# ssmit1986/BayesianInference

Measured on AMD Instinct MI355X. Metric: GP log-marg-lik evals/sec at N=32768, d=8; Cholesky TFLOP/s vs fp64 peak, higher is better.
Workload: dtype f64

## Files before the change

bayesianinference_amd/csrc/gp_trsv.h:

```cpp
#pragma once
#include "gp_kernels.h"

namespace gphip {

constexpr int TRSV_MAXR = 4;
constexpr int TRSV_CHAIN = 8;
constexpr int TRSV_SPIN_LIMIT = 1 << 24;
#ifndef TRSV_TILE_BACKOFF
#define TRSV_TILE_BACKOFF 6
#endif

template <typename T>
struct TrsvArgs {
    const T* A; int R128;
    const T* W;
    const T* P;
    const T* B;
    T* X;
    T* Xc;
    T* S;
    long ldx;
    int nt, nrhs, back;
    int dbg;
    unsigned int* ticket;
    long long* trace;
    int* abort_flag;
};

template <typename T> struct TrsvBits;
template <> struct TrsvBits<double> {
    typedef unsigned long long u;
    static __device__ __forceinline__ bool pending(double v) { return __double_as_longlong(v) == -1ll; }
};
template <> struct TrsvBits<float> {
    typedef unsigned int u;
    static __device__ __forceinline__ bool pending(float v) { return __float_as_int(v) == -1; }
};

template <typename T, int MODE, typename Src>
__device__ __forceinline__ void trsv_fetch(Src src, int nrhs, T* dst, int lane, int* abort_flag) {
    T va[2 * TRSV_MAXR];
    int spins = 0;
    auto give_up = [&]() -> bool {
        if ((++spins & 255) != 0) return false;
        if (__hip_atomic_load(abort_flag, __ATOMIC_RELAXED, __HIP_MEMORY_SCOPE_AGENT) != 0) return true;
        if (spins > TRSV_SPIN_LIMIT) { __hip_atomic_store(abort_flag, 1, __ATOMIC_RELAXED, __HIP_MEMORY_SCOPE_AGENT); return true; }
        return false;
    };
    auto load_set = [&](T (&v)[2 * TRSV_MAXR]) {
#pragma unroll
        for (int r = 0; r < TRSV_MAXR; ++r)
            if (r < nrhs) {
                const T* p = src(r);
                if (MODE == 0) {
                    v[2 * r] = p[lane];
                    v[2 * r + 1] = p[64 + lane];
                } else {
                    v[2 * r] = __hip_atomic_load(p + lane, __ATOMIC_RELAXED, __HIP_MEMORY_SCOPE_AGENT);
                    v[2 * r + 1] = __hip_atomic_load(p + 64 + lane, __ATOMIC_RELAXED, __HIP_MEMORY_SCOPE_AGENT);
                }
            }
    };
    auto complete = [&](const T (&v)[2 * TRSV_MAXR]) -> bool {
        bool bad = false;
#pragma unroll
        for (int r = 0; r < TRSV_MAXR; ++r)
            if (r < nrhs) bad = bad || TrsvBits<T>::pending(v[2 * r]) || TrsvBits<T>::pending(v[2 * r + 1]);
        return __all(!bad);
    };
    load_set(va);
    if (MODE != 0) {
        while (__builtin_expect(!complete(va), 0)) {
            if (MODE == 1) __builtin_amdgcn_s_sleep(TRSV_TILE_BACKOFF);
            load_set(va);
            if (give_up()) break;
        }
    }
#pragma unroll
    for (int r = 0; r < TRSV_MAXR; ++r)
        if (r < nrhs) {
            dst[r * TB + lane] = va[2 * r];
            dst[r * TB + 64 + lane] = va[2 * r + 1];
        }
}

template <typename T, bool BACK> struct TrsvBlk {
    static constexpr int NC = BACK ? 4 : 8, NR = BACK ? 8 : 4;
    T a[BACK ? 4 : 8][BACK ? 8 : 4];
};
template <typename T, bool BACK>
__device__ __forceinline__ void trsv_load_tile(TrsvBlk<T, BACK>& m, const T* __restrict__ tile, int lo, int ob) {
    constexpr int NC = TrsvBlk<T, BACK>::NC, NR = TrsvBlk<T, BACK>::NR;
    const int c0 = BACK ? 4 * ob : 8 * lo, r0 = BACK ? 8 * lo : 4 * ob;
#pragma unroll
    for (int cc = 0; cc < NC; ++cc) {
        const T* p = tile + (long)(c0 + cc) * TB + r0;
#pragma unroll
        for (int rr = 0; rr < NR; ++rr) m.a[cc][rr] = p[rr];
    }
}

template <typename T, bool BACK>
__device__ __forceinline__ void trsv_settle(TrsvBlk<T, BACK>& m) {
    asm volatile("s_waitcnt vmcnt(0)" ::: "memory");
#pragma unroll
    for (int cc = 0; cc < TrsvBlk<T, BACK>::NC; ++cc)
#pragma unroll
        for (int rr = 0; rr < TrsvBlk<T, BACK>::NR; ++rr) asm volatile("" : "+v"(m.a[cc][rr]));
}

template <int CTRL> __device__ __forceinline__ double trsv_dpp(double v) {
    const int lo = __builtin_amdgcn_update_dpp(0, __double2loint(v), CTRL, 0xF, 0xF, true);
    const int hi = __builtin_amdgcn_update_dpp(0, __double2hiint(v), CTRL, 0xF, 0xF, true);
    return __hiloint2double(hi, lo);
}
template <int CTRL> __device__ __forceinline__ float trsv_dpp(float v) {
    return __int_as_float(__builtin_amdgcn_update_dpp(0, __float_as_int(v), CTRL, 0xF, 0xF, true));
}
template <typename T> __device__ __forceinline__ T trsv_row16_sum(T v) {
    v += trsv_dpp<0xB1>(v);
    v += trsv_dpp<0x4E>(v);
    v += trsv_dpp<0x141>(v);
    v += trsv_dpp<0x140>(v);
    return v;
}

template <typename T, bool BACK>
__device__ __forceinline__ void trsv_matvec(const TrsvBlk<T, BACK>& m, const T* x, int lo, T (&y)[4]) {
    T xv[8];
#pragma unroll
    for (int k = 0; k < 8; ++k) xv[k] = x[lo * 8 + k];
    if constexpr (!BACK) {
#pragma unroll
        for (int rr = 0; rr < 4; ++rr) {
            T acc = (T)0;
#pragma unroll
            for (int cc = 0; cc < 8; ++cc) acc = __builtin_fma(m.a[cc][rr], xv[cc], acc);
            y[rr] = acc;
        }
    } else {
#pragma unroll
        for (int cc = 0; cc < 4; ++cc) {
            T acc = (T)0;
#pragma unroll
            for (int rr = 0; rr < 8; ++rr) acc = __builtin_fma(m.a[cc][rr], xv[rr], acc);
            y[cc] = acc;
        }
    }
#pragma unroll
    for (int k = 0; k < 4; ++k) y[k] = trsv_row16_sum(y[k]);
}

template <typename T, bool BACK> struct TrsvHalf {
    static constexpr int NC = BACK ? 2 : 8, NR = BACK ? 8 : 2;
    T a[BACK ? 2 : 8][BACK ? 8 : 2];
};
template <typename T, bool BACK>
__device__ __forceinline__ void trsv_load_half(TrsvHalf<T, BACK>& m, const T* __restrict__ tile, int lo, int ob, int hf) {
    constexpr int NC = TrsvHalf<T, BACK>::NC, NR = TrsvHalf<T, BACK>::NR;
    const int c0 = BACK ? 64 * hf + 2 * ob : 8 * lo, r0 = BACK ? 8 * lo : 64 * hf + 2 * ob;
#pragma unroll
    for (int cc = 0; cc < NC; ++cc) {
        const T* p = tile + (long)(c0 + cc) * TB + r0;
#pragma unroll
        for (int rr = 0; rr < NR; ++rr) m.a[cc][rr] = p[rr];
    }
}
template <typename T, bool BACK>
__device__ __forceinline__ void trsv_settle_half(TrsvHalf<T, BACK>& m) {
    asm volatile("s_waitcnt vmcnt(0)" ::: "memory");
#pragma unroll
    for (int cc = 0; cc < TrsvHalf<T, BACK>::NC; ++cc)
#pragma unroll
        for (int rr = 0; rr < TrsvHalf<T, BACK>::NR; ++rr) asm volatile("" : "+v"(m.a[cc][rr]));
}
template <typename T, bool BACK>
__device__ __forceinline__ void trsv_half_fma(const TrsvHalf<T, BACK>& m, const T* x, int lo, bool negate, T (&y)[2]) {
    T xv[8];
#pragma unroll
    for (int k = 0; k < 8; ++k) xv[k] = negate ? -x[lo * 8 + k] : x[lo * 8 + k];
    if constexpr (!BACK) {
#pragma unroll
        for (int cc = 0; cc < 8; ++cc)
#pragma unroll
            for (int rr = 0; rr < 2; ++rr) y[rr] = __builtin_fma(m.a[cc][rr], xv[cc], y[rr]);
    } else {
#pragma unroll
        for (int rr = 0; rr < 8; ++rr)
#pragma unroll
            for (int cc = 0; cc < 2; ++cc) y[cc] = __builtin_fma(m.a[cc][rr], xv[rr], y[cc]);
    }
}

template <typename T>
__global__ __launch_bounds__(256) void trsv_prep_kernel(const T* __restrict__ A, int R128, const T* __restrict__ W, T* __restrict__ P, int nt, int back) {
    __shared__ T As[16][TB + 4], Bs[16][TB + 4];
    const int b = blockIdx.x, gap = (int)blockIdx.y + 1, tid = threadIdx.x, tx = tid & 15, ty = tid >> 4;
    if (back ? b > nt - 1 - gap : b < gap) return;
    P += (long)blockIdx.y * nt * TS;
    const T* Lt = A + tile_index(back ? b + gap : b, back ? b : b - gap, R128) * TS;
    const T* Wb = W + (long)b * TS;
    const T* Am = back ? Lt : Wb;
    const T* Bm = back ? Wb : Lt;
    T c[8][8];
#pragma unroll
    for (int i = 0; i < 8; ++i)
#pragma unroll
        for (int j = 0; j < 8; ++j) c[i][j] = (T)0;
    for (int k0 = 0; k0 < TB; k0 += 16) {
        for (int idx = tid; idx < 16 * TB; idx += 256) {
            const int kk = idx >> 7, r = idx & 127;
            As[kk][r] = Am[(long)(k0 + kk) * TB + r];
        }
        for (int idx = tid; idx < 16 * TB; idx += 256) {
            const int cc = idx >> 4, kk = idx & 15;
            Bs[kk][cc] = Bm[(long)cc * TB + k0 + kk];
        }
        __syncthreads();
#pragma unroll 4
        for (int kk = 0; kk < 16; ++kk) {
            T av[8], bv[8];
#pragma unroll
            for (int i = 0; i < 8; ++i) { av[i] = As[kk][8 * ty + i]; bv[i] = Bs[kk][8 * tx + i]; }
#pragma unroll
            for (int i = 0; i < 8; ++i)
#pragma unroll
                for (int j = 0; j < 8; ++j) c[i][j] = __builtin_fma(av[i], bv[j], c[i][j]);
        }
        __syncthreads();
    }
    T* Pb = P + (long)b * TS;
#pragma unroll
    for (int j = 0; j < 8; ++j)
#pragma unroll
        for (int i = 0; i < 8; ++i) Pb[(long)(8 * tx + j) * TB + 8 * ty + i] = c[i][j];
}

constexpr int TRSV_THREADS = 512;

template <typename T, bool BACK>
__global__ __launch_bounds__(TRSV_THREADS, 1) void trsv_dataflow_kernel(TrsvArgs<T> g) {
    constexpr int NC = TrsvBlk<T, BACK>::NC, NR = TrsvBlk<T, BACK>::NR;
    extern __shared__ double trsv_lds_raw[];
    __shared__ unsigned int s_q;
    T* xs = reinterpret_cast<T*>(trsv_lds_raw);
    T* ss = xs + TRSV_MAXR * TB;
    const int tid = threadIdx.x, lane = tid & 63, wave = tid >> 6;
    const int lo = tid & 15, ob = tid >> 4;
    const int nt = g.nt, nrhs = g.nrhs;
    auto blk = [&](int K) { return BACK ? nt - 1 - K : K; };
    const T* Xpoll = (g.dbg & 64) ? g.Xc : g.X;
    auto sslot = [&](int I, int K) { return g.S + ((long)I * (I - 1) / 2 + K) * nrhs * TB; };
    auto ltile = [&](int I, int K) {
        const int bi = blk(I), bk = blk(K);
        return g.A + tile_index(bi > bk ? bi : bk, bi > bk ? bk : bi, g.R128) * TS;
    };

    if ((int)blockIdx.x < 2 * TRSV_CHAIN) {
        TrsvHalf<T, BACK> w, p1, p2;
        const int hf = (int)blockIdx.x & 1;
        T* xs2 = ss + TRSV_MAXR * TB;
        for (int K = (int)blockIdx.x >> 1; K < nt; K += TRSV_CHAIN) {
            const int b = blk(K);
            long long* tr = (g.trace && hf == 0) ? g.trace + (long)K * 8 : nullptr;
            long long st[8];
            auto stamp = [&](int k) { if (tr) st[k] = wall_clock64(); };
            stamp(0);
            if (tr) st[6] = clock64();
            trsv_load_half<T, BACK>(w, g.W + (long)b * TS, lo, ob, hf);
            if (K > 0) trsv_load_half<T, BACK>(p1, g.P + (long)b * TS, lo, ob, hf);
            if (K > 1) trsv_load_half<T, BACK>(p2, g.P + ((long)nt + b) * TS, lo, ob, hf);
            trsv_settle_half(w);
            trsv_settle_half(p1);
            trsv_settle_half(p2);
            if (wave == 1) {
                if (K >= 3 && !(g.dbg & 1)) trsv_fetch<T, 2>([&](int r) { return sslot(K, K - 3) + (long)r * TB; }, nrhs, ss, lane, g.abort_flag);
                else trsv_fetch<T, 0>([&](int r) { return g.B + (long)r * g.ldx + (long)b * TB; }, nrhs, ss, lane, g.abort_flag);
            }
            if (wave == 2 && K > 1)
                trsv_fetch<T, 1>([&](int r) { return g.X + (long)r * g.ldx + (long)blk(K - 2) * TB; }, nrhs, xs2, lane, g.abort_flag);
            __syncthreads();
            stamp(2);
            T y[TRSV_MAXR][2];
#pragma unroll
            for (int r = 0; r < TRSV_MAXR; ++r) {
                y[r][0] = y[r][1] = (T)0;
                if (r < nrhs) {
                    trsv_half_fma<T, BACK>(w, ss + r * TB, lo, false, y[r]);
                    if (K > 1) trsv_half_fma<T, BACK>(p2, xs2 + r * TB, lo, true, y[r]);
                }
            }
            stamp(3);
            if (wave == 0 && K > 0)
                trsv_fetch<T, 2>([&](int r) { return g.Xc + (long)r * g.ldx + (long)blk(K - 1) * TB; }, nrhs, xs, lane, g.abort_flag);
            stamp(1);
            __syncthreads();
            stamp(4);
#pragma unroll
            for (int r = 0; r < TRSV_MAXR; ++r)
                if (r < nrhs) {
                    if (K > 0) trsv_half_fma<T, BACK>(p1, xs + r * TB, lo, true, y[r]);
                    y[r][0] = trsv_row16_sum(y[r][0]);
                    y[r][1] = trsv_row16_sum(y[r][1]);
                    if (lo == 0) {
                        T* oc = g.Xc + (long)r * g.ldx + (long)b * TB + 64 * hf + 2 * ob;
                        T* ox = g.X + (long)r * g.ldx + (long)b * TB + 64 * hf + 2 * ob;
                        __hip_atomic_store(oc, y[r][0], __ATOMIC_RELAXED, __HIP_MEMORY_SCOPE_AGENT);
                        __hip_atomic_store(oc + 1, y[r][1], __ATOMIC_RELAXED, __HIP_MEMORY_SCOPE_AGENT);
                        __hip_atomic_store(ox, y[r][0], __ATOMIC_RELAXED, __HIP_MEMORY_SCOPE_AGENT);
                        __hip_atomic_store(ox + 1, y[r][1], __ATOMIC_RELAXED, __HIP_MEMORY_SCOPE_AGENT);
                    }
                }
            stamp(5);
            if (tr) {
                st[7] = clock64();
                if (tid == 0)
                    for (int k = 0; k < 8; ++k) tr[k] = st[k];
            }
            __syncthreads();
        }
        return;
    }

    auto tile_out = [&](const TrsvBlk<T, BACK>& cur, int I, int K) {
        T* out = sslot(I, K);
        for (int r = 0; r < nrhs; ++r) {
            T y[4];
            trsv_matvec<T, BACK>(cur, xs + r * TB, lo, y);
            if (lo == 0) {
#pragma unroll
                for (int k = 0; k < 4; ++k)
                    __hip_atomic_store(out + (long)r * TB + ob * 4 + k, ss[r * TB + ob * 4 + k] - y[k], __ATOMIC_RELAXED, __HIP_MEMORY_SCOPE_AGENT);
            }
        }
    };
    if ((int)blockIdx.x < 3 * TRSV_CHAIN) {
        TrsvBlk<T, BACK> cur;
        for (int K = (int)blockIdx.x - 2 * TRSV_CHAIN; K + 3 < nt; K += TRSV_CHAIN) {
            const int I = K + 3;
            trsv_load_tile<T, BACK>(cur, ltile(I, K), lo, ob);
            trsv_settle(cur);
            if (wave == 0) trsv_fetch<T, 1>([&](int r) { return g.X + (long)r * g.ldx + (long)blk(K) * TB; }, nrhs, xs, lane, g.abort_flag);
            if (wave == 1) {
                if (K > 0) trsv_fetch<T, 1>([&](int r) { return sslot(I, K - 1) + (long)r * TB; }, nrhs, ss, lane, g.abort_flag);
                else trsv_fetch<T, 0>([&](int r) { return g.B + (long)r * g.ldx + (long)blk(I) * TB; }, nrhs, ss, lane, g.abort_flag);
            }
            __syncthreads();
            tile_out(cur, I, K);
            __syncthreads();
        }
        return;
    }

    if (nt < 5) return;
    const long ntasks = (long)(nt - 4) * (nt - 3) / 2;
    auto take = [&]() -> long {
        __syncthreads();
        if (tid == 0) s_q = atomicAdd(g.ticket, 1u) + 1u;
        __syncthreads();
        return (long)s_q;
    };
    auto decode = [&](long q, int& I, int& K) {
        const double bq = (double)(2 * nt - 7);
        int k = (int)((bq - sqrt(bq * bq - 8.0 * (double)q)) * 0.5);
        if (k < 0) k = 0;
        if (k > nt - 5) k = nt - 5;
        while (k + 1 <= nt - 5 && (long)(k + 1) * (nt - 4) - (long)(k + 1) * k / 2 <= q) ++k;
        while (k > 0 && (long)k * (nt - 4) - (long)k * (k - 1) / 2 > q) --k;
        K = __builtin_amdgcn_readfirstlane(k);
        I = __builtin_amdgcn_readfirstlane(k + 4 + (int)(q - ((long)k * (nt - 4) - (long)k * (k - 1) / 2)));
    };
    TrsvBlk<T, BACK> ta, tb;
    long q = take();
    if (q >= ntasks) return;
    int I, K;
    decode(q, I, K);
    trsv_load_tile<T, BACK>(ta, ltile(I, K), lo, ob);
    auto process = [&](TrsvBlk<T, BACK>& cur, TrsvBlk<T, BACK>& nxt) -> bool {
        const long qn = take();
        int In = 0, Kn = 0;
        if (qn < ntasks) {
            decode(qn, In, Kn);
            trsv_load_tile<T, BACK>(nxt, ltile(In, Kn), lo, ob);
        }
        if (wave == 0) trsv_fetch<T, 1>([&](int r) { return Xpoll + (long)r * g.ldx + (long)blk(K) * TB; }, nrhs, xs, lane, g.abort_flag);
        if (wave == 1) {
            if (K > 0) trsv_fetch<T, 1>([&](int r) { return sslot(I, K - 1) + (long)r * TB; }, nrhs, ss, lane, g.abort_flag);
            else trsv_fetch<T, 0>([&](int r) { return g.B + (long)r * g.ldx + (long)blk(I) * TB; }, nrhs, ss, lane, g.abort_flag);
        }
        trsv_settle(cur);
        trsv_settle(nxt);
        __syncthreads();
        tile_out(cur, I, K);
        I = In; K = Kn;
        return qn < ntasks;
    };
    for (;;) {
        if (!process(ta, tb)) return;
        if (!process(tb, ta)) return;
    }
}

template <typename T>
__global__ void rows_to_vblock_kernel(const T* __restrict__ rows, int mc, long npad, T* __restrict__ V, long mpad) {
    const long j = (long)blockIdx.x * blockDim.x + threadIdx.x;
    if (j >= npad) return;
    for (long t = 0; t < mpad; ++t) V[j * mpad + t] = t < mc ? rows[t * npad + j] : (T)0;
}
template <typename T>
__global__ void vblock_to_rows_kernel(const T* __restrict__ V, long mpad, int mc, long npad, T* __restrict__ rows) {
    const long j = (long)blockIdx.x * blockDim.x + threadIdx.x;
    if (j >= npad) return;
    for (int t = 0; t < mc; ++t) rows[(long)t * npad + j] = V[j * mpad + t];
}

template <typename T>
__global__ __launch_bounds__(256) void w128_to_w64_kernel(const T* __restrict__ W128, T* __restrict__ W64, long slot_stride = 0) {
    const int j = blockIdx.x, b = j >> 1, q = j & 1;
    const T* src = W128 + (long)blockIdx.y * slot_stride + (long)b * TS + (long)(q * 64) * TB + q * 64;
    T* dst = W64 + (long)blockIdx.y * slot_stride + (long)j * 4096;
    for (int idx = threadIdx.x; idx < 4096; idx += 256) {
        const int c = idx >> 6, r = idx & 63;
        dst[idx] = src[(long)c * TB + r];
    }
}

constexpr size_t trsv_lds_bytes(size_t es) { return (size_t)(3 * TRSV_MAXR * TB) * es; }

}
```

bayesianinference_amd/csrc/gphip.hip:

```cpp
#include "gp_kernels.h"
#include "gp_trsv.h"
#include "rccl_dyn.h"
#include "rtc_dyn.h"

#include <hip/hip_ext.h>

#include <algorithm>
#include <chrono>
#include <cctype>
#include <cmath>
#include <cstdio>
#include <cstdlib>
#include <cstring>
#include <mutex>
#include <string>
#include <vector>

#include "../../include/gphip.h"

using namespace gphip;

namespace {

constexpr double LOG_TWO_PI = 1.8378770664093454835606594728112;
// ... 99 lines not shown
    Buf dA, dXs, dW;
    Buf dDinv;
    Buf dW64;
    unsigned long w64_gen = ~0ul;
    Buf dLT, dW64T;
    unsigned long lt_gen = ~0ul;
    Buf dInvEll, dSlotp, dPartial, dRes, dInfo;
    Buf hInvEll, hSlotp, hRes, hInfo;
    int panel = 4, profile = 0, swizzle = 1, max_slots = 256, lookahead = 1;
    int supertile = 2;
    int latency_gemm = 1;
    static constexpr int latency_tiles = 256;
    int latency_max_nt = 48;
    int dataflow = 1, dataflow_max_nt = 96;
    int dataflow_max_slots = -1;
    int dataflow_max_tasks = 34000;
    int dataflow_fine_nt = 96;
    int panel_left = -1;
    int fuse_option = 1;
    int grad_potri = 1;
    int grad_batch_slots = 0;
    int grad_batch_max_n = 7168;
    int grad_batch_last = 0, grad_batch_route = 0;
    Buf dKinvB;
    int predict_df_max_nt = 256;
    int predict_df = 2048;
    int panel_wide = 1;
    int thin_tiles = 1;
    int debug_fail_alloc = 0;
    int debug_abort_word = 0;
    int dataflow_tail = 64;
    bool fused_eval = false;
    bool theta_packed = false;
    bool want_w = false;
    bool want_u = false;
    unsigned long u_gen = ~0ul;
    Buf dFlags;
    Buf dTicket;
    const char* abort_unread = nullptr;
    unsigned long long ticket_base = 0;
    int epoch = 0;
    bool fitted = false;
    std::vector<double> theta_fit;
    unsigned long ws_gen = 0, fit_gen = ~0ul, fit_id = 0;
    double logdet_fit = 0, mu_fit = 0, kappa_fit = 0;
    Buf dV, dXsT, dXsS;
    Buf dMean, dVar;
    Buf dPart;
    int64_t vcap = 0;
    Buf dAlpha;
    Buf dTrsvX;
    Buf dRows;
    Buf dTrsvP;
    unsigned long trsvp_gen = ~0ul;
    int trsv = 1;
    int ncu = 0;
    Buf dKinv;
    Buf dGacc;
    Buf dLoo;
    std::vector<ProfRec> recs;
    std::vector<hipEvent_t> pool;
    double acc_ms[GPHIP_NCLASS] = {0}, acc_n[GPHIP_NCLASS] = {0}, acc_flops[GPHIP_NCLASS] = {0},
           acc_bytes[GPHIP_NCLASS] = {0};
    std::string err;
    struct gphip_group* group = nullptr;
    int shard_min_n = 16384;
    hipStream_t cstream = nullptr;
    Buf packed[3];
    Buf dScal8;
    Buf drain_buf;
    int last_issue_us = 0;
    int debug_fail_hip = 0;
    int fit_rank = 0, fit_world = 0;
    bool in_group_call = false;
    int replicate_factor = 0;
    int share_local_panels = 1;
    Buf dOwn;
    void* dist_base = nullptr;
    std::vector<long> dist_adj;
    Buf dDistAdj;
    int lay_rank = -1, lay_world = 0, lay_panel = 0, lay_full = -1;
    void* ws_override = nullptr;
    bool dist_fit = false;
    Buf dZ;
    bool null_fit = false;
    const double *pw_mean_host = nullptr, *pw_nug_host = nullptr;
    const double *pw_mean_test = nullptr, *pw_nug_test = nullptr;
    long pw_test_stride = 0;
    Buf dPwMean, dPwNug;
    bool pw_mean_on = false, pw_nug_on = false;
    Buf dPwMeanT, dPwNugT;
    std::vector<double> null_diag, null_mean_test;
    std::vector<double> fit_pw_mean, fit_pw_nug;
    bool fit_pw = false;
    gphip_ctx* joint = nullptr;
    Buf dJZ;
    Buf dJPart;
    Buf dJOut;
    int joint_split = 0;
    int joint_nsplit = 0;
    Buf dXgPart;
    Buf dXgOut;
    int predict_grad_split = 0;
    int predict_grad_nsplit = 0;
    int predict_grad_chunk = 0;
    int predict_grad_chunk_last = 0;
    int extend_logpdf_us = 0, extend_create_us = 0, extend_assemble_us = 0, extend_derive_us = 0;
// ... 1460 lines not shown
    const size_t np = h->ngacc, nwg = (size_t)grid.x * grid.y, need = nwg * np * 8 * (size_t)G;
    a.gpart = nullptr; a.np = (int)np; a.ws_off = (int)((lds + 7) / 8);
    if (st) st->gpart = (long)(nwg * np);
    if (np == 0 || 4 * np * 8 > 8192) return lds;
    if (h->dGpart.grow(need) != hipSuccess) { (void)hipGetLastError(); return lds; }
    a.gpart = h->dGpart.as<double>();
    return (size_t)a.ws_off * 8 + 4 * np * 8;
}
template <typename T>
void grad_rows_finish(gphip_ctx* h, const GradArgs<T>& a, dim3 grid, int G = 1, const GradStride* st = nullptr) {
    if (a.gpart)
        hipLaunchKernelGGL(grad_finish_kernel, dim3((unsigned)a.np, (unsigned)G), dim3(256), 0, h->cs, (const double*)a.gpart,
                           (long)grid.x * grid.y, a.np, a.gacc, st ? st->gpart : 0l, st ? st->gacc : 0l);
}

template <typename T>
void launch_grad(gphip_ctx* h, GradArgs<T>& a, dim3 grid, int G = 1, GradStride* st = nullptr) {
    if (h->custom) {
        const size_t lds = grad_rows<T>(h, a, grid, (size_t)((a.d > KB_LDS_MAXD ? 0 : a.d) + 1) * TB * sizeof(T), G, st);
        for (int s = 0; s < G; ++s) {
            GradArgs<T> as = G == 1 ? a : GradSlots<T>{a, *st}.at(s);
            const double* cp = h->dCustomP.as<double>() + (size_t)s * h->ncp;
            int ncp = h->ncp;
            void* params[] = {&as, &cp, &ncp};
            (void)hipModuleLaunchKernel(h->f_cgrad, grid.x, grid.y, grid.z, 256, 1, 1, (unsigned)lds, h->cs, params, nullptr);
        }
        grad_rows_finish<T>(h, a, grid, G, st);
        return;
    }
    if (a.d > KB_LDS_MAXD) {
        a.ks = h->ks; a.xs2 = (const T*)h->dXs2.p;
        const size_t lds = grad_rows<T>(h, a, grid, (size_t)TB * sizeof(T), G, st);
        for (a.d0 = 0; a.d0 < a.d; a.d0 += 32) {
            GRAD_LAUNCH(grad_reduce_general_kernel<T>, grad_reduce_general_slots_kernel<T>);
            grad_rows_finish<T>(h, a, grid, G, st);
        }
        a.d0 = 0;
        return;
    }
    if (h->kt == 0 || h->kt == 1) {
        const size_t lds = grad_rows<T>(h, a, grid, (size_t)(a.d + 1) * TB * sizeof(T), G, st);
        if (h->kt == 0) launch_grad_kt<T, 0>(h, a, grid, lds, G, st);
        else launch_grad_kt<T, 1>(h, a, grid, lds, G, st);
    } else {
        a.ks = h->ks; a.xs2 = (const T*)h->dXs2.p;
        const size_t lds = grad_rows<T>(h, a, grid, (size_t)(4 * a.d + 1) * TB * sizeof(T), G, st);
        GRAD_LAUNCH(grad_reduce_general_kernel<T>, grad_reduce_general_slots_kernel<T>);
    }
    grad_rows_finish<T>(h, a, grid, G, st);
}
#undef GRAD_LAUNCH

size_t trsv_pass_elems(const gphip_ctx* h, int nrhs) {
    return (size_t)nrhs * ((size_t)2 * h->Npad + (size_t)TB * (size_t)(h->Nt * (h->Nt - 1) / 2 + 1)) + 64 / h->es;
}
bool trsv_ok(gphip_ctx* h, int nrhs) {
    if (!h->trsv || nrhs < 1 || nrhs > TRSV_MAXR || h->Nt > 512 || h->dist_world > 0 || h->ws_override) return false;
    const size_t bytes = ((size_t)TRSV_MAXR * h->Npad + 2 * trsv_pass_elems(h, TRSV_MAXR)) * h->es;
    if (h->dTrsvX.grow(bytes) != hipSuccess || h->dTrsvP.grow((size_t)4 * h->Nt * TS * h->es) != hipSuccess) {
        (void)hipGetLastError();
        return false;
    }
    return true;
}
template <typename T> T* trsv_input(gphip_ctx* h) { return (T*)h->dTrsvX.p; }
template <typename T> T* trsv_pass(gphip_ctx* h, int nrhs, int pass) { return (T*)h->dTrsvX.p + (size_t)TRSV_MAXR * h->Npad + (size_t)pass * trsv_pass_elems(h, nrhs); }

template <typename T>
int queue_trsv_fill(gphip_ctx* h, int nrhs, int npasses) {
    HIPCHK(hipMemsetAsync(trsv_pass<T>(h, nrhs, 0), 0xFF, (size_t)npasses * trsv_pass_elems(h, nrhs) * sizeof(T), h->stream));
    return GPHIP_OK;
}

template <typename T>
int queue_trsv(gphip_ctx* h, const T* B, int pass, int nrhs, bool back, T** Xout) {
    const int nt = (int)h->Nt;
    if (h->trsvp_gen != h->ws_gen) {
        for (int dir = 0; dir < 2; ++dir)
            hipLaunchKernelGGL(trsv_prep_kernel<T>, dim3((unsigned)nt, 2), dim3(256), 0, h->stream, (const T*)h->dA.p, (int)h->R, (const T*)h->dW.p,
                               (T*)h->dTrsvP.p + (size_t)dir * 2 * nt * TS, nt, dir);
        h->trsvp_gen = h->ws_gen;
    }
    T* base = trsv_pass<T>(h, nrhs, pass);
    TrsvArgs<T> g{};
    g.A = (const T*)h->dA.p; g.R128 = (int)h->R; g.W = (const T*)h->dW.p; g.B = B; g.ldx = (long)h->Npad;
    g.P = (const T*)h->dTrsvP.p + (size_t)(back ? 1 : 0) * 2 * nt * TS;
    g.X = base; g.Xc = base + (size_t)nrhs * h->Npad; g.S = base + (size_t)2 * nrhs * h->Npad;
    g.ticket = reinterpret_cast<unsigned int*>(g.S + (size_t)nrhs * TB * (size_t)(nt * (nt - 1) / 2 + 1));
    g.nt = nt; g.nrhs = nrhs; g.back = back ? 1 : 0; g.dbg = 0;
    g.abort_flag = reinterpret_cast<int*>(h->dTicket.as<unsigned long long>() + 1);
    const long ntasks = nt >= 5 ? (long)(nt - 4) * (nt - 3) / 2 : 0;
    const long grid = std::min<long>((long)h->ncu, 3 * TRSV_CHAIN + ntasks);
    ProfScope ps(h, 2, 0.0, (double)h->slot_elems * sizeof(T));
    abort_hook(h, 3);
    if (!h->abort_unread) h->abort_unread = "single-vector substitution timed out (set option trsv=0 and report)";
    if (back) hipLaunchKernelGGL((trsv_dataflow_kernel<T, true>), dim3((unsigned)grid), dim3(TRSV_THREADS), trsv_lds_bytes(sizeof(T)), h->stream, g);
    else hipLaunchKernelGGL((trsv_dataflow_kernel<T, false>), dim3((unsigned)grid), dim3(TRSV_THREADS), trsv_lds_bytes(sizeof(T)), h->stream, g);
    *Xout = g.X;
    return GPHIP_OK;
}

template <typename T>
int queue_trsv_solve(gphip_ctx* h, const std::vector<double>& b, std::vector<float>& b32, int nr, void** x) {
    const void* src = b.data();
    if constexpr (sizeof(T) == 4) { b32.assign(b.begin(), b.end()); src = b32.data(); }
    HIPCHK(hipMemcpyAsync(h->dTrsvX.p, src, b.size() * sizeof(T), hipMemcpyHostToDevice, h->stream));
    T *x0 = nullptr, *x1 = nullptr;
    int rc = queue_trsv_fill<T>(h, nr, 2);
    if (!rc) rc = queue_trsv<T>(h, trsv_input<T>(h), 0, nr, false, &x0);
    if (!rc) rc = queue_trsv<T>(h, x0, 1, nr, true, &x1);
    *x = x1;
    return rc;
}

template <typename T>
void queue_rows_vblock(gphip_ctx* h, void* rows, int64_t mc, int64_t mpad, bool to_v) {
    const unsigned gx = (unsigned)((h->Npad + 255) / 256);
    if (to_v) hipLaunchKernelGGL(rows_to_vblock_kernel<T>, dim3(gx), dim3(256), 0, h->stream, (const T*)rows, (int)mc, (long)h->Npad, (T*)h->dV.p, (long)mpad);
    else hipLaunchKernelGGL(vblock_to_rows_kernel<T>, dim3(gx), dim3(256), 0, h->stream, (const T*)h->dV.p, (long)mpad, (int)mc, (long)h->Npad, (T*)rows);
}

template <typename T>
int queue_alpha(gphip_ctx* h) {
    const int64_t mpad = TB, Npad = h->Npad;
    if (trsv_ok(h, 1)) {
        T *z = trsv_input<T>(h), *x = nullptr;
        hipLaunchKernelGGL(gather_rhs_row_kernel<T>, dim3((unsigned)((Npad + 255) / 256)), dim3(256), 0, h->stream, (const T*)h->dA.p,
                           (int)h->R, 0, (int)Npad, z, 1l);
        int rc = queue_trsv_fill<T>(h, 1, 1);
        if (!rc) rc = queue_trsv<T>(h, z, 0, 1, true, &x);
        if (rc) return rc;
        HIPCHK(hipMemcpyAsync(h->dAlpha.p, x, (size_t)Npad * sizeof(T), hipMemcpyDeviceToDevice, h->stream));
        return GPHIP_OK;
    }
    HIPCHK(hipMemsetAsync(h->dV.p, 0, (size_t)mpad * Npad * sizeof(T), h->stream));
    hipLaunchKernelGGL(gather_rhs_row_kernel<T>, dim3((unsigned)((Npad + 255) / 256)), dim3(256), 0, h->stream, (const T*)h->dA.p,
                       (int)h->R, 0, (int)Npad, (T*)h->dV.p, (long)mpad);
    queue_backward_rows<T>(h, mpad);
    HIPCHK(hipMemcpy2DAsync(h->dAlpha.p, sizeof(T), h->dV.p, (size_t)mpad * sizeof(T), sizeof(T), (size_t)Npad,
                            hipMemcpyDeviceToDevice, h->stream));
    return GPHIP_OK;
}

template <typename T>
GradArgs<T> grad_args(gphip_ctx* h, const void* Kinv, long ld, int64_t c0, int64_t mc) {
// ... 1551 lines not shown
```

Baseline: 5.533.

## Restructure dataflow triangular solve to process 128-row block pairs per chain step

```diff
diff --git a/bayesianinference_amd/csrc/gp_trsv.h b/bayesianinference_amd/csrc/gp_trsv.h
--- a/bayesianinference_amd/csrc/gp_trsv.h
+++ b/bayesianinference_amd/csrc/gp_trsv.h
@@ -4,7 +4,13 @@
 namespace gphip {
 
 constexpr int TRSV_MAXR = 4;
-constexpr int TRSV_CHAIN = 8;
+#ifndef TRSV_CHAIN
+#define TRSV_CHAIN 8
+#endif
+#ifndef TRSV_CHAIN_BIG
+#define TRSV_CHAIN_BIG 4
+#endif
+constexpr int TRSV_BIG_NT = 160;
 constexpr int TRSV_SPIN_LIMIT = 1 << 24;
 #ifndef TRSV_TILE_BACKOFF
 #define TRSV_TILE_BACKOFF 6
@@ -21,11 +27,26 @@
     T* S;
     long ldx;
     int nt, nrhs, back;
+    int nch;
     int dbg;
     unsigned int* ticket;
     long long* trace;
     int* abort_flag;
 };
+
+__host__ __device__ __forceinline__ long trsv_sum_slot(int I, int Jc) {
+    const long JI = I >> 1, ib = I & 1;
+    return (JI - 1) * (JI - 2 + ib) + Jc;
+}
+__host__ __device__ __forceinline__ long trsv_sum_slots(int nt) { return nt < 5 ? 0 : trsv_sum_slot(nt, 0); }
+__host__ __device__ __forceinline__ long trsv_tile_tasks(int nt) {
+    if (nt < 7) return 0;
+    const long m = 2 * nt - 12, nj = (m + 3) / 4;
+    return nj * m - 2 * nj * (nj - 1);
+}
+__host__ __device__ __forceinline__ int trsv_chain_quads(int nt) { return nt >= TRSV_BIG_NT ? TRSV_CHAIN_BIG : TRSV_CHAIN; }
+
+template <typename T> __host__ __device__ constexpr int trsv_xpad(int i) { return i + (i >> 3) * (int)(16 / sizeof(T)); }
 
 template <typename T> struct TrsvBits;
 template <> struct TrsvBits<double> {
@@ -37,9 +58,10 @@
     static __device__ __forceinline__ bool pending(float v) { return __float_as_int(v) == -1; }
 };
 
-template <typename T, int MODE, typename Src>
+template <typename T, int MODE, int NV, int DS, bool PAD, typename Src>
 __device__ __forceinline__ void trsv_fetch(Src src, int nrhs, T* dst, int lane, int* abort_flag) {
-    T va[2 * TRSV_MAXR];
+    constexpr int PER = NV / 64;
+    T va[PER * TRSV_MAXR];
     int spins = 0;
     auto give_up = [&]() -> bool {
         if ((++spins & 255) != 0) return false;
@@ -47,25 +69,26 @@
         if (spins > TRSV_SPIN_LIMIT) { __hip_atomic_store(abort_flag, 1, __ATOMIC_RELAXED, __HIP_MEMORY_SCOPE_AGENT); return true; }
         return false;
     };
-    auto load_set = [&](T (&v)[2 * TRSV_MAXR]) {
+    auto load_set = [&](T (&v)[PER * TRSV_MAXR]) {
 #pragma unroll
         for (int r = 0; r < TRSV_MAXR; ++r)
             if (r < nrhs) {
                 const T* p = src(r);
-                if (MODE == 0) {
-                    v[2 * r] = p[lane];
-                    v[2 * r + 1] = p[64 + lane];
-                } else {
-                    v[2 * r] = __hip_atomic_load(p + lane, __ATOMIC_RELAXED, __HIP_MEMORY_SCOPE_AGENT);
-                    v[2 * r + 1] = __hip_atomic_load(p + 64 + lane, __ATOMIC_RELAXED, __HIP_MEMORY_SCOPE_AGENT);
+#pragma unroll
+                for (int k = 0; k < PER; ++k) {
+                    if (MODE == 0) v[PER * r + k] = p[64 * k + lane];
+                    else v[PER * r + k] = __hip_atomic_load(p + 64 * k + lane, __ATOMIC_RELAXED, __HIP_MEMORY_SCOPE_AGENT);
                 }
             }
     };
-    auto complete = [&](const T (&v)[2 * TRSV_MAXR]) -> bool {
+    auto complete = [&](const T (&v)[PER * TRSV_MAXR]) -> bool {
         bool bad = false;
 #pragma unroll
         for (int r = 0; r < TRSV_MAXR; ++r)
-            if (r < nrhs) bad = bad || TrsvBits<T>::pending(v[2 * r]) || TrsvBits<T>::pending(v[2 * r + 1]);
+            if (r < nrhs) {
+#pragma unroll
+                for (int k = 0; k < PER; ++k) bad = bad || TrsvBits<T>::pending(v[PER * r + k]);
+            }
         return __all(!bad);
     };
     load_set(va);
@@ -79,8 +102,8 @@
 #pragma unroll
     for (int r = 0; r < TRSV_MAXR; ++r)
         if (r < nrhs) {
-            dst[r * TB + lane] = va[2 * r];
-            dst[r * TB + 64 + lane] = va[2 * r + 1];
+#pragma unroll
+            for (int k = 0; k < PER; ++k) dst[PAD ? r * trsv_xpad<T>(DS) + trsv_xpad<T>(64 * k + lane) : r * DS + 64 * k + lane] = va[PER * r + k];
         }
 }
 
@@ -89,9 +112,9 @@
     T a[BACK ? 4 : 8][BACK ? 8 : 4];
 };
 template <typename T, bool BACK>
-__device__ __forceinline__ void trsv_load_tile(TrsvBlk<T, BACK>& m, const T* __restrict__ tile, int lo, int ob) {
+__device__ __forceinline__ void trsv_load_tile(TrsvBlk<T, BACK>& m, const T* __restrict__ tile, int lo, int oo) {
     constexpr int NC = TrsvBlk<T, BACK>::NC, NR = TrsvBlk<T, BACK>::NR;
-    const int c0 = BACK ? 4 * ob : 8 * lo, r0 = BACK ? 8 * lo : 4 * ob;
+    const int c0 = BACK ? oo : 8 * lo, r0 = BACK ? 8 * lo : oo;
 #pragma unroll
     for (int cc = 0; cc < NC; ++cc) {
         const T* p = tile + (long)(c0 + cc) * TB + r0;
@@ -129,7 +152,7 @@
 __device__ __forceinline__ void trsv_matvec(const TrsvBlk<T, BACK>& m, const T* x, int lo, T (&y)[4]) {
     T xv[8];
 #pragma unroll
-    for (int k = 0; k < 8; ++k) xv[k] = x[lo * 8 + k];
+    for (int k = 0; k < 8; ++k) xv[k] = x[trsv_xpad<T>(lo * 8) + k];
     if constexpr (!BACK) {
 #pragma unroll
         for (int rr = 0; rr < 4; ++rr) {
@@ -178,7 +201,7 @@
 __device__ __forceinline__ void trsv_half_fma(const TrsvHalf<T, BACK>& m, const T* x, int lo, bool negate, T (&y)[2]) {
     T xv[8];
 #pragma unroll
-    for (int k = 0; k < 8; ++k) xv[k] = negate ? -x[lo * 8 + k] : x[lo * 8 + k];
+    for (int k = 0; k < 8; ++k) xv[k] = negate ? -x[trsv_xpad<T>(lo * 8) + k] : x[trsv_xpad<T>(lo * 8) + k];
     if constexpr (!BACK) {
 #pragma unroll
         for (int cc = 0; cc < 8; ++cc)
@@ -193,20 +216,8 @@
 }
 
 template <typename T>
-__global__ __launch_bounds__(256) void trsv_prep_kernel(const T* __restrict__ A, int R128, const T* __restrict__ W, T* __restrict__ P, int nt, int back) {
-    __shared__ T As[16][TB + 4], Bs[16][TB + 4];
-    const int b = blockIdx.x, gap = (int)blockIdx.y + 1, tid = threadIdx.x, tx = tid & 15, ty = tid >> 4;
-    if (back ? b > nt - 1 - gap : b < gap) return;
-    P += (long)blockIdx.y * nt * TS;
-    const T* Lt = A + tile_index(back ? b + gap : b, back ? b : b - gap, R128) * TS;
-    const T* Wb = W + (long)b * TS;
-    const T* Am = back ? Lt : Wb;
-    const T* Bm = back ? Wb : Lt;
-    T c[8][8];
-#pragma unroll
-    for (int i = 0; i < 8; ++i)
-#pragma unroll
-        for (int j = 0; j < 8; ++j) c[i][j] = (T)0;
+__device__ __forceinline__ void trsv_mm128(const T* __restrict__ Am, const T* __restrict__ Bm, T (&c)[8][8], T (&As)[16][TB + 4], T (&Bs)[16][TB + 4]) {
+    const int tid = threadIdx.x, tx = tid & 15, ty = tid >> 4;
     for (int k0 = 0; k0 < TB; k0 += 16) {
         for (int idx = tid; idx < 16 * TB; idx += 256) {
             const int kk = idx >> 7, r = idx & 127;
@@ -229,6 +240,23 @@
         }
         __syncthreads();
     }
+}
+
+template <typename T>
+__global__ __launch_bounds__(256) void trsv_prep_kernel(const T* __restrict__ A, int R128, const T* __restrict__ W, T* __restrict__ P, int nt, int back) {
+    __shared__ T As[16][TB + 4], Bs[16][TB + 4];
+    const int b = blockIdx.x, gap = (int)blockIdx.y + 1, tid = threadIdx.x, tx = tid & 15, ty = tid >> 4;
+    const int mb = back ? nt - 1 - b : b;
+    if (mb < gap || (gap == 3 && (mb & 1) == 0)) return;
+    P += (long)blockIdx.y * nt * TS;
+    const T* Lt = A + tile_index(back ? b + gap : b, back ? b : b - gap, R128) * TS;
+    const T* Wb = W + (long)b * TS;
+    T c[8][8];
+#pragma unroll
+    for (int i = 0; i < 8; ++i)
+#pragma unroll
+        for (int j = 0; j < 8; ++j) c[i][j] = (T)0;
+    trsv_mm128<T>(back ? Lt : Wb, back ? Wb : Lt, c, As, Bs);
     T* Pb = P + (long)b * TS;
 #pragma unroll
     for (int j = 0; j < 8; ++j)
@@ -236,49 +264,90 @@
         for (int i = 0; i < 8; ++i) Pb[(long)(8 * tx + j) * TB + 8 * ty + i] = c[i][j];
 }
 
+template <typename T>
+__global__ __launch_bounds__(256) void trsv_prep_pair_kernel(const T* __restrict__ W, T* P, int nt, int back) {
+    __shared__ T As[16][TB + 4], Bs[16][TB + 4];
+    const int J = blockIdx.x, t = blockIdx.y, tid = threadIdx.x, tx = tid & 15, ty = tid >> 4;
+    if (t > 0 && J == 0) return;
+    const int ra = back ? nt - 1 - 2 * J : 2 * J, rb = back ? ra - 1 : ra + 1;
+    const T* X = P + (long)rb * TS;
+    const T* Y = t == 0 ? W + (long)ra * TS : P + ((long)(t - 1) * nt + ra) * TS;
+    T* D = t == 0 ? P + ((long)2 * nt + ra) * TS : P + ((long)t * nt + rb) * TS;
+    T c[8][8];
+#pragma unroll
+    for (int i = 0; i < 8; ++i)
+#pragma unroll
+        for (int j = 0; j < 8; ++j) c[i][j] = (T)0;
+    trsv_mm128<T>(back ? Y : X, back ? X : Y, c, As, Bs);
+#pragma unroll
+    for (int j = 0; j < 8; ++j)
+#pragma unroll
+        for (int i = 0; i < 8; ++i) {
+            T* d = D + (long)(8 * tx + j) * TB + 8 * ty + i;
+            *d = t == 0 ? c[i][j] : *d - c[i][j];
+        }
+}
+
 constexpr int TRSV_THREADS = 512;
 
 template <typename T, bool BACK>
 __global__ __launch_bounds__(TRSV_THREADS, 1) void trsv_dataflow_kernel(TrsvArgs<T> g) {
-    constexpr int NC = TrsvBlk<T, BACK>::NC, NR = TrsvBlk<T, BACK>::NR;
     extern __shared__ double trsv_lds_raw[];
     __shared__ unsigned int s_q;
+    constexpr int XB = trsv_xpad<T>(TB);
     T* xs = reinterpret_cast<T*>(trsv_lds_raw);
-    T* ss = xs + TRSV_MAXR * TB;
+    T* ss = xs + TRSV_MAXR * 2 * XB;
+    T* sa = ss + TRSV_MAXR * XB;
     const int tid = threadIdx.x, lane = tid & 63, wave = tid >> 6;
     const int lo = tid & 15, ob = tid >> 4;
-    const int nt = g.nt, nrhs = g.nrhs;
+    const int nt = g.nt, nrhs = g.nrhs, nch = g.nch;
     auto blk = [&](int K) { return BACK ? nt - 1 - K : K; };
-    const T* Xpoll = (g.dbg & 64) ? g.Xc : g.X;
-    auto sslot = [&](int I, int K) { return g.S + ((long)I * (I - 1) / 2 + K) * nrhs * TB; };
+    auto sslot = [&](int I, int Jc) { return g.S + trsv_sum_slot(I, Jc) * nrhs * TB; };
     auto ltile = [&](int I, int K) {
         const int bi = blk(I), bk = blk(K);
         return g.A + tile_index(bi > bk ? bi : bk, bi > bk ? bk : bi, g.R128) * TS;
     };
-
-    if ((int)blockIdx.x < 2 * TRSV_CHAIN) {
-        TrsvHalf<T, BACK> w, p1, p2;
-        const int hf = (int)blockIdx.x & 1;
-        T* xs2 = ss + TRSV_MAXR * TB;
-        for (int K = (int)blockIdx.x >> 1; K < nt; K += TRSV_CHAIN) {
-            const int b = blk(K);
-            long long* tr = (g.trace && hf == 0) ? g.trace + (long)K * 8 : nullptr;
+    const long ldx = g.ldx;
+    auto xsrc = [&](const T* X, int K) {
+        const T* p = X + (long)blk(K) * TB;
+        return [p, ldx](int r) { return p + (long)r * ldx; };
+    };
+
+    if ((int)blockIdx.x < 4 * nch) {
+        TrsvHalf<T, BACK> w, cc, q1, q2;
+        const int ib = ((int)blockIdx.x >> 1) & 1, hf = (int)blockIdx.x & 1;
+        T* Xc2 = g.Xc + (long)nrhs * g.ldx;
+        const T* Xpoll = ib ? Xc2 : g.Xc;
+        for (int J = (int)blockIdx.x >> 2; 2 * J + ib < nt; J += nch) {
+            const int I = 2 * J + ib, rI = blk(I), ra = blk(2 * J);
+            long long* tr = (g.trace && hf == 0 && ib == 0) ? g.trace + (long)J * 8 : nullptr;
             long long st[8];
             auto stamp = [&](int k) { if (tr) st[k] = wall_clock64(); };
             stamp(0);
             if (tr) st[6] = clock64();
-            trsv_load_half<T, BACK>(w, g.W + (long)b * TS, lo, ob, hf);
-            if (K > 0) trsv_load_half<T, BACK>(p1, g.P + (long)b * TS, lo, ob, hf);
-            if (K > 1) trsv_load_half<T, BACK>(p2, g.P + ((long)nt + b) * TS, lo, ob, hf);
+            trsv_load_half<T, BACK>(w, g.W + (long)rI * TS, lo, ob, hf);
+            if (ib) trsv_load_half<T, BACK>(cc, g.P + ((long)2 * nt + ra) * TS, lo, ob, hf);
+            if (J > 0) {
+                trsv_load_half<T, BACK>(q1, g.P + ((long)ib * nt + rI) * TS, lo, ob, hf);
+                trsv_load_half<T, BACK>(q2, g.P + ((long)(ib + 1) * nt + rI) * TS, lo, ob, hf);
+            }
             trsv_settle_half(w);
-            trsv_settle_half(p1);
-            trsv_settle_half(p2);
+            trsv_settle_half(cc);
+            trsv_settle_half(q1);
+            trsv_settle_half(q2);
             if (wave == 1) {
-                if (K >= 3 && !(g.dbg & 1)) trsv_fetch<T, 2>([&](int r) { return sslot(K, K - 3) + (long)r * TB; }, nrhs, ss, lane, g.abort_flag);
-                else trsv_fetch<T, 0>([&](int r) { return g.B + (long)r * g.ldx + (long)b * TB; }, nrhs, ss, lane, g.abort_flag);
-            }
-            if (wave == 2 && K > 1)
-                trsv_fetch<T, 1>([&](int r) { return g.X + (long)r * g.ldx + (long)blk(K - 2) * TB; }, nrhs, xs2, lane, g.abort_flag);
+                if (J >= 2 && !(g.dbg & 1)) trsv_fetch<T, 2, 128, 128, true>([&](int r) { return sslot(I, J - 2) + (long)r * TB; }, nrhs, ss, lane, g.abort_flag);
+                else trsv_fetch<T, 0, 128, 128, true>(xsrc(g.B, I), nrhs, ss, lane, g.abort_flag);
+            }
+            if (wave == 2 && ib) {
+                if (J >= 2 && !(g.dbg & 1)) trsv_fetch<T, 2, 128, 128, true>([&](int r) { return sslot(I - 1, J - 2) + (long)r * TB; }, nrhs, sa, lane, g.abort_flag);
+                else trsv_fetch<T, 0, 128, 128, true>(xsrc(g.B, I - 1), nrhs, sa, lane, g.abort_flag);
+            }
+            if (J > 0) {
+                if (wave == 0) trsv_fetch<T, 2, 128, 2 * TB, true>(xsrc(Xpoll, 2 * J - 2), nrhs, xs, lane, g.abort_flag);
+                if (wave == 3) trsv_fetch<T, 2, 128, 2 * TB, true>(xsrc(Xpoll, 2 * J - 1), nrhs, xs + XB, lane, g.abort_flag);
+            }
+            stamp(1);
             __syncthreads();
             stamp(2);
             T y[TRSV_MAXR][2];
@@ -286,29 +355,29 @@
             for (int r = 0; r < TRSV_MAXR; ++r) {
                 y[r][0] = y[r][1] = (T)0;
                 if (r < nrhs) {
-                    trsv_half_fma<T, BACK>(w, ss + r * TB, lo, false, y[r]);
-                    if (K > 1) trsv_half_fma<T, BACK>(p2, xs2 + r * TB, lo, true, y[r]);
+                    trsv_half_fma<T, BACK>(w, ss + r * XB, lo, false, y[r]);
+                    if (ib) trsv_half_fma<T, BACK>(cc, sa + r * XB, lo, true, y[r]);
                 }
             }
             stamp(3);
-            if (wave == 0 && K > 0)
-                trsv_fetch<T, 2>([&](int r) { return g.Xc + (long)r * g.ldx + (long)blk(K - 1) * TB; }, nrhs, xs, lane, g.abort_flag);
-            stamp(1);
-            __syncthreads();
             stamp(4);
 #pragma unroll
             for (int r = 0; r < TRSV_MAXR; ++r)
                 if (r < nrhs) {
-                    if (K > 0) trsv_half_fma<T, BACK>(p1, xs + r * TB, lo, true, y[r]);
+                    if (J > 0) {
+                        trsv_half_fma<T, BACK>(q2, xs + r * 2 * XB, lo, true, y[r]);
+                        trsv_half_fma<T, BACK>(q1, xs + r * 2 * XB + XB, lo, true, y[r]);
+                    }
                     y[r][0] = trsv_row16_sum(y[r][0]);
                     y[r][1] = trsv_row16_sum(y[r][1]);
                     if (lo == 0) {
-                        T* oc = g.Xc + (long)r * g.ldx + (long)b * TB + 64 * hf + 2 * ob;
-                        T* ox = g.X + (long)r * g.ldx + (long)b * TB + 64 * hf + 2 * ob;
-                        __hip_atomic_store(oc, y[r][0], __ATOMIC_RELAXED, __HIP_MEMORY_SCOPE_AGENT);
-                        __hip_atomic_store(oc + 1, y[r][1], __ATOMIC_RELAXED, __HIP_MEMORY_SCOPE_AGENT);
-                        __hip_atomic_store(ox, y[r][0], __ATOMIC_RELAXED, __HIP_MEMORY_SCOPE_AGENT);
-                        __hip_atomic_store(ox + 1, y[r][1], __ATOMIC_RELAXED, __HIP_MEMORY_SCOPE_AGENT);
+                        const long o = (long)r * g.ldx + (long)rI * TB + 64 * hf + 2 * ob;
+                        __hip_atomic_store(g.Xc + o, y[r][0], __ATOMIC_RELAXED, __HIP_MEMORY_SCOPE_AGENT);
+                        __hip_atomic_store(g.Xc + o + 1, y[r][1], __ATOMIC_RELAXED, __HIP_MEMORY_SCOPE_AGENT);
+                        __hip_atomic_store(Xc2 + o, y[r][0], __ATOMIC_RELAXED, __HIP_MEMORY_SCOPE_AGENT);
+                        __hip_atomic_store(Xc2 + o + 1, y[r][1], __ATOMIC_RELAXED, __HIP_MEMORY_SCOPE_AGENT);
+                        __hip_atomic_store(g.X + o, y[r][0], __ATOMIC_RELAXED, __HIP_MEMORY_SCOPE_AGENT);
+                        __hip_atomic_store(g.X + o + 1, y[r][1], __ATOMIC_RELAXED, __HIP_MEMORY_SCOPE_AGENT);
                     }
                 }
             stamp(5);
@@ -322,77 +391,96 @@
         return;
     }
 
-    auto tile_out = [&](const TrsvBlk<T, BACK>& cur, int I, int K) {
-        T* out = sslot(I, K);
-        for (int r = 0; r < nrhs; ++r) {
-            T y[4];
-            trsv_matvec<T, BACK>(cur, xs + r * TB, lo, y);
-            if (lo == 0) {
-#pragma unroll
-                for (int k = 0; k < 4; ++k)
-                    __hip_atomic_store(out + (long)r * TB + ob * 4 + k, ss[r * TB + ob * 4 + k] - y[k], __ATOMIC_RELAXED, __HIP_MEMORY_SCOPE_AGENT);
-            }
-        }
-    };
-    if ((int)blockIdx.x < 3 * TRSV_CHAIN) {
+    const int ts = wave >> 2, o4 = 4 * (ob & 15);
+    auto load_task = [&](TrsvBlk<T, BACK>& m, int I, int hh, int Jc) { trsv_load_tile<T, BACK>(m, ltile(I, 2 * Jc + ts), lo, 64 * hh + o4); };
+    auto task_inputs = [&](int I, int hh, int Jc) {
+        if (wave == 0) trsv_fetch<T, 1, 128, 2 * TB, true>(xsrc(g.X, 2 * Jc), nrhs, xs, lane, g.abort_flag);
+        if (wave == 4) trsv_fetch<T, 1, 128, 2 * TB, true>(xsrc(g.X, 2 * Jc + 1), nrhs, xs + XB, lane, g.abort_flag);
+        if (wave == 1) {
+            if (Jc > 0) trsv_fetch<T, 1, 64, 64, false>([&](int r) { return sslot(I, Jc - 1) + (long)r * TB + 64 * hh; }, nrhs, ss, lane, g.abort_flag);
+            else trsv_fetch<T, 0, 64, 64, false>([&](int r) { return g.B + (long)r * g.ldx + (long)blk(I) * TB + 64 * hh; }, nrhs, ss, lane, g.abort_flag);
+        }
+    };
+    auto task_out = [&](const TrsvBlk<T, BACK>& cur, int I, int hh, int Jc) {
+        T y[TRSV_MAXR][4];
+#pragma unroll
+        for (int r = 0; r < TRSV_MAXR; ++r)
+            if (r < nrhs) {
+                trsv_matvec<T, BACK>(cur, xs + r * 2 * XB + ts * XB, lo, y[r]);
+                if (lo == 0 && ts == 1) {
+#pragma unroll
+                    for (int k = 0; k < 4; ++k) sa[r * 64 + o4 + k] = y[r][k];
+                }
+            }
+        __syncthreads();
+        if (lo == 0 && ts == 0) {
+            T* out = sslot(I, Jc) + 64 * hh + o4;
+#pragma unroll
+            for (int r = 0; r < TRSV_MAXR; ++r)
+                if (r < nrhs) {
+#pragma unroll
+                    for (int k = 0; k < 4; ++k)
+                        __hip_atomic_store(out + (long)r * TB + k, (ss[r * 64 + o4 + k] - y[r][k]) - sa[r * 64 + o4 + k], __ATOMIC_RELAXED, __HIP_MEMORY_SCOPE_AGENT);
+                }
+        }
+    };
+    if ((int)blockIdx.x < 8 * nch) {
         TrsvBlk<T, BACK> cur;
-        for (int K = (int)blockIdx.x - 2 * TRSV_CHAIN; K + 3 < nt; K += TRSV_CHAIN) {
-            const int I = K + 3;
-            trsv_load_tile<T, BACK>(cur, ltile(I, K), lo, ob);
+        const int f = (int)blockIdx.x - 4 * nch, ib = (f >> 1) & 1, hh = f & 1;
+        for (int J = f >> 2; 2 * J + ib < nt; J += nch) {
+            if (J < 2) continue;
+            const int I = 2 * J + ib, Jc = J - 2;
+            load_task(cur, I, hh, Jc);
             trsv_settle(cur);
-            if (wave == 0) trsv_fetch<T, 1>([&](int r) { return g.X + (long)r * g.ldx + (long)blk(K) * TB; }, nrhs, xs, lane, g.abort_flag);
-            if (wave == 1) {
-                if (K > 0) trsv_fetch<T, 1>([&](int r) { return sslot(I, K - 1) + (long)r * TB; }, nrhs, ss, lane, g.abort_flag);
-                else trsv_fetch<T, 0>([&](int r) { return g.B + (long)r * g.ldx + (long)blk(I) * TB; }, nrhs, ss, lane, g.abort_flag);
-            }
+            task_inputs(I, hh, Jc);
             __syncthreads();
-            tile_out(cur, I, K);
+            task_out(cur, I, hh, Jc);
             __syncthreads();
         }
         return;
     }
 
-    if (nt < 5) return;
-    const long ntasks = (long)(nt - 4) * (nt - 3) / 2;
+    const long ntasks = trsv_tile_tasks(nt);
+    if (ntasks == 0) return;
     auto take = [&]() -> long {
         __syncthreads();
         if (tid == 0) s_q = atomicAdd(g.ticket, 1u) + 1u;
         __syncthreads();
         return (long)s_q;
     };
-    auto decode = [&](long q, int& I, int& K) {
-        const double bq = (double)(2 * nt - 7);
-        int k = (int)((bq - sqrt(bq * bq - 8.0 * (double)q)) * 0.5);
-        if (k < 0) k = 0;
-        if (k > nt - 5) k = nt - 5;
-        while (k + 1 <= nt - 5 && (long)(k + 1) * (nt - 4) - (long)(k + 1) * k / 2 <= q) ++k;
-        while (k > 0 && (long)k * (nt - 4) - (long)k * (k - 1) / 2 > q) --k;
-        K = __builtin_amdgcn_readfirstlane(k);
-        I = __builtin_amdgcn_readfirstlane(k + 4 + (int)(q - ((long)k * (nt - 4) - (long)k * (k - 1) / 2)));
+    const long m = 2 * nt - 12;
+    auto decode = [&](long q, int& I, int& hh, int& Jc) {
+        const double bq = (double)(m + 2);
+        const long jmax = (m + 3) / 4 - 1;
+        long j = (long)((bq - sqrt(bq * bq - 8.0 * (double)q)) * 0.25);
+        if (j < 0) j = 0;
+        if (j > jmax) j = jmax;
+        while (j + 1 <= jmax && (j + 1) * m - 2 * (j + 1) * j <= q) ++j;
+        while (j > 0 && j * m - 2 * j * (j - 1) > q) --j;
+        const int h = (int)(4 * j + 12 + (q - (j * m - 2 * j * (j - 1))));
+        Jc = __builtin_amdgcn_readfirstlane((int)j);
+        I = __builtin_amdgcn_readfirstlane(h >> 1);
+        hh = __builtin_amdgcn_readfirstlane(h & 1);
     };
     TrsvBlk<T, BACK> ta, tb;
     long q = take();
     if (q >= ntasks) return;
-    int I, K;
-    decode(q, I, K);
-    trsv_load_tile<T, BACK>(ta, ltile(I, K), lo, ob);
+    int I, hh, Jc;
+    decode(q, I, hh, Jc);
+    load_task(ta, I, hh, Jc);
     auto process = [&](TrsvBlk<T, BACK>& cur, TrsvBlk<T, BACK>& nxt) -> bool {
         const long qn = take();
-        int In = 0, Kn = 0;
+        int In = 0, hn = 0, Jn = 0;
         if (qn < ntasks) {
-            decode(qn, In, Kn);
-            trsv_load_tile<T, BACK>(nxt, ltile(In, Kn), lo, ob);
-        }
-        if (wave == 0) trsv_fetch<T, 1>([&](int r) { return Xpoll + (long)r * g.ldx + (long)blk(K) * TB; }, nrhs, xs, lane, g.abort_flag);
-        if (wave == 1) {
-            if (K > 0) trsv_fetch<T, 1>([&](int r) { return sslot(I, K - 1) + (long)r * TB; }, nrhs, ss, lane, g.abort_flag);
-            else trsv_fetch<T, 0>([&](int r) { return g.B + (long)r * g.ldx + (long)blk(I) * TB; }, nrhs, ss, lane, g.abort_flag);
-        }
+            decode(qn, In, hn, Jn);
+            load_task(nxt, In, hn, Jn);
+        }
+        task_inputs(I, hh, Jc);
         trsv_settle(cur);
         trsv_settle(nxt);
         __syncthreads();
-        tile_out(cur, I, K);
-        I = In; K = Kn;
+        task_out(cur, I, hh, Jc);
+        I = In; hh = hn; Jc = Jn;
         return qn < ntasks;
     };
     for (;;) {
@@ -425,6 +513,6 @@
     }
 }
 
-constexpr size_t trsv_lds_bytes(size_t es) { return (size_t)(3 * TRSV_MAXR * TB) * es; }
-
-}
+constexpr size_t trsv_lds_bytes(size_t es) { return (size_t)(4 * TRSV_MAXR) * (TB * es + TB / 8 * 16); }
+
+}
diff --git a/bayesianinference_amd/csrc/gphip.hip b/bayesianinference_amd/csrc/gphip.hip
--- a/bayesianinference_amd/csrc/gphip.hip
+++ b/bayesianinference_amd/csrc/gphip.hip
@@ -175,7 +175,7 @@
     Buf dTrsvX;
     Buf dRows;
     Buf dTrsvP;
-    unsigned long trsvp_gen = ~0ul;
+    unsigned long trsvp_gen[2] = {~0ul, ~0ul};
     int trsv = 1;
     int ncu = 0;
     Buf dKinv;
@@ -1742,12 +1742,12 @@
 #undef GRAD_LAUNCH
 
 size_t trsv_pass_elems(const gphip_ctx* h, int nrhs) {
-    return (size_t)nrhs * ((size_t)2 * h->Npad + (size_t)TB * (size_t)(h->Nt * (h->Nt - 1) / 2 + 1)) + 64 / h->es;
+    return (size_t)nrhs * ((size_t)3 * h->Npad + (size_t)TB * (size_t)(trsv_sum_slots((int)h->Nt) + 1)) + 64 / h->es;
 }
 bool trsv_ok(gphip_ctx* h, int nrhs) {
-    if (!h->trsv || nrhs < 1 || nrhs > TRSV_MAXR || h->Nt > 512 || h->dist_world > 0 || h->ws_override) return false;
+    if (!h->trsv || nrhs < 1 || nrhs > TRSV_MAXR || h->Nt > 512 || h->dist_world > 0 || h->ws_override || h->ncu <= 8 * TRSV_CHAIN) return false;
     const size_t bytes = ((size_t)TRSV_MAXR * h->Npad + 2 * trsv_pass_elems(h, TRSV_MAXR)) * h->es;
-    if (h->dTrsvX.grow(bytes) != hipSuccess || h->dTrsvP.grow((size_t)4 * h->Nt * TS * h->es) != hipSuccess) {
+    if (h->dTrsvX.grow(bytes) != hipSuccess || h->dTrsvP.grow((size_t)6 * h->Nt * TS * h->es) != hipSuccess) {
         (void)hipGetLastError();
         return false;
     }
@@ -1765,22 +1765,22 @@
 template <typename T>
 int queue_trsv(gphip_ctx* h, const T* B, int pass, int nrhs, bool back, T** Xout) {
     const int nt = (int)h->Nt;
-    if (h->trsvp_gen != h->ws_gen) {
-        for (int dir = 0; dir < 2; ++dir)
-            hipLaunchKernelGGL(trsv_prep_kernel<T>, dim3((unsigned)nt, 2), dim3(256), 0, h->stream, (const T*)h->dA.p, (int)h->R, (const T*)h->dW.p,
-                               (T*)h->dTrsvP.p + (size_t)dir * 2 * nt * TS, nt, dir);
-        h->trsvp_gen = h->ws_gen;
+    const int dir = back ? 1 : 0;
+    if (h->trsvp_gen[dir] != h->ws_gen) {
+        T* P = (T*)h->dTrsvP.p + (size_t)dir * 3 * nt * TS;
+        hipLaunchKernelGGL(trsv_prep_kernel<T>, dim3((unsigned)nt, 3), dim3(256), 0, h->stream, (const T*)h->dA.p, (int)h->R, (const T*)h->dW.p, P, nt, dir);
+        if (nt >= 2) hipLaunchKernelGGL(trsv_prep_pair_kernel<T>, dim3((unsigned)(nt / 2), 3), dim3(256), 0, h->stream, (const T*)h->dW.p, P, nt, dir);
+        h->trsvp_gen[dir] = h->ws_gen;
     }
     T* base = trsv_pass<T>(h, nrhs, pass);
     TrsvArgs<T> g{};
     g.A = (const T*)h->dA.p; g.R128 = (int)h->R; g.W = (const T*)h->dW.p; g.B = B; g.ldx = (long)h->Npad;
-    g.P = (const T*)h->dTrsvP.p + (size_t)(back ? 1 : 0) * 2 * nt * TS;
-    g.X = base; g.Xc = base + (size_t)nrhs * h->Npad; g.S = base + (size_t)2 * nrhs * h->Npad;
-    g.ticket = reinterpret_cast<unsigned int*>(g.S + (size_t)nrhs * TB * (size_t)(nt * (nt - 1) / 2 + 1));
-    g.nt = nt; g.nrhs = nrhs; g.back = back ? 1 : 0; g.dbg = 0;
+    g.P = (const T*)h->dTrsvP.p + (size_t)dir * 3 * nt * TS;
+    g.X = base; g.Xc = base + (size_t)nrhs * h->Npad; g.S = base + (size_t)3 * nrhs * h->Npad;
+    g.ticket = reinterpret_cast<unsigned int*>(g.S + (size_t)nrhs * TB * (size_t)(trsv_sum_slots(nt) + 1));
+    g.nt = nt; g.nrhs = nrhs; g.back = back ? 1 : 0; g.nch = trsv_chain_quads(nt); g.dbg = 0;
     g.abort_flag = reinterpret_cast<int*>(h->dTicket.as<unsigned long long>() + 1);
-    const long ntasks = nt >= 5 ? (long)(nt - 4) * (nt - 3) / 2 : 0;
-    const long grid = std::min<long>((long)h->ncu, 3 * TRSV_CHAIN + ntasks);
+    const long grid = std::min<long>((long)h->ncu, 8 * g.nch + trsv_tile_tasks(nt));
     ProfScope ps(h, 2, 0.0, (double)h->slot_elems * sizeof(T));
     abort_hook(h, 3);
     if (!h->abort_unread) h->abort_unread = "single-vector substitution timed out (set option trsv=0 and report)";
```

New measurement: 5.527, median of 2. Within noise of the previous version (-0.1%).
